# fukangl/SMG-multimodal-grasping

Hardware: AMD Instinct MI355X
Metric: affordance fwd+bwd passes/sec (16-rot 224^2 RGB-D) (higher is better)
Workload: dtype f32; 1 GPU; 16 rot x 224^2 (S=640): fwd + Huber + bwd + Adam per GPU per step; reinforcement_net style 0; 17 trunk passes; fp32; leg=headline, rotations=16, input_size=640, parallelism=dp1

## Files before the change

### smg-multimodal-grasping_amd/csrc/backward.hip

```cpp
#include "engine.h"

int do_backward(smg_engine* e, const smg_net* net, const float* dq, hipStream_t st, int phases, bool elem_head) {
    if (!e->have_fwd) return fail(-22, "smg_backward without a preceding smg_forward");
    if (!net->grads) return fail(-22, "net.grads is NULL");
    if (phases == 2 && !e->bw_phase0_done)
        return fail(-22, "smg_backward_phase(1) must follow smg_backward_phase(0) of the same forward");
    if ((phases & 1) && e->bw_phase0_done)
        return fail(-22, "smg_backward / smg_backward_phase(0) while the second half of a two-phase backward is still due (run phase 1 or a new forward)");
    const Layout& L = *e->L;
    const TrunkRef& T = L.trunk[e->f_trunk];
    const HeadRef& Hd = L.head[e->f_head];
    const int NS = e->f_streams, NP = e->f_pairs;
    const float* P = net->params;
    float* Gr = net->grads;
    const Plane p4 = e->p_blk[3];
    const bool ph_a = phases & 1, ph_b = phases & 2;
    if (ph_a) {
        for (int r = 0; r < kStatRep; ++r) HIP_OK(hipMemsetAsync(e->bstat + (size_t)r * kStatRepStride, 0, 2 * e->bstat_span * sizeof(double), st));
    }
    const bool split16 = e->prec == 0 && kSplitOp == 3;
    if (ph_a && split16) HIP_OK(hipMemsetAsync(e->gamax, 0, (size_t)e->gamax_words * sizeof(unsigned), st));
    const hipStream_t s2 = (e->prof || e->serialize) ? st : e->side;
    auto fork = [&](hipEvent_t ev) -> int {
        HIP_OK(hipEventRecord(ev, st));
        HIP_OK(hipStreamWaitEvent(s2, ev, 0));
        return 0;
    };
    const bool gs_materialised = split16 || NS > 4;
    auto gs_on_side = [&](const Plane& pl) { return split16 && !e->generic3x3 && pl.HW <= 1600 && NS <= 4; };
    auto fused_gsrc = [&](int b, const DenseLayerRef& d) {
        return grad_src(e, e->G[b], kBlockCtot[b], e->X[b], kBlockCtot[b], e->st_X[b], d.cin, nullptr);
    };
    auto launch_gs_apply = [&](int b, int i, hipStream_t cs, float* GSb, const GradSrc& fused) {
        const Plane pl = e->p_blk[b];
        BnBwdApplyArgs a{};
        a.src = fused; a.src.xtab = stat_table(e, e->sx_tab[b], e->max_streams, kBlockCtot[b], T.layers[b][i].cin);
        a.pl = pl; a.C = kGrowth;
        a.out = GSb; a.ldo = kGrowth; a.amax = split16 ? gamax_of(e, b, i, 0) : nullptr;
        PREC_DISPATCH(e, launch_kernel(e, bn_bwd_apply_kernel<PREC>, dim3((pl.HWp + bn_apply_rows(PREC) - 1) / bn_apply_rows(PREC), NS), dim3(256), 0, cs,
                                       K_OTHER, 0, ESZ(e) * NS * pl.HW * 3 * kGrowth, false, a));
    };

    auto norm1_src = [&](int b, int i, int c0) {
        const DenseLayerRef& d = T.layers[b][i];
        return act_src(e, e->X[b], kBlockCtot[b], e->st_X[b], c0, P + d.n1.w, P + d.n1.b, stat_table(e, e->sx_tab[b], e->max_streams, kBlockCtot[b]), asc_n1(e, b, i));
    };
    auto norm2_src = [&](int b, int i) {
        const DenseLayerRef& d = T.layers[b][i];
        return act_src(e, el(e, e->Bt, e->bt_off[b][i]), kBottleneck, e->st_Bt[b][i], 0, P + d.n2.w, P + d.n2.b,
                       !e->generic3x3 ? stat_table(e, e->sb_tab[b][i], e->max_streams, kBottleneck) : StatTab{}, asc_n2(e, b, i));
    };

    PartialTiles tiles(e->part_floats, NS, e->deterministic);

    if (ph_a) {
    {
        ValueBwdArgs a;
        a.h1 = head_norm1_src(e, Hd, P); a.p4 = p4; a.w2p = e->packed_f + e->pk_head1;
        a.dq = dq; a.out_ch = e->head_out; a.OH = e->OH; a.OW = e->OW; a.dh1 = e->DH1;
        a.st = stat_sink_bwd(e, e->st_H1, 0); a.aff = affine_sink(Gr, Hd.n1); a.dw2 = Gr + Hd.c1.w;
        const bool dense = !elem_head && (e->head_bwd == 2 || (e->head_bwd == 0 && e->f_dense_dq));
        if (!dense) {
// ... 149 lines not shown
        }
        HIP_OK(hipMemcpyAsync(buf, src, (size_t)elems * (e->prec ? 2 : 4), hipMemcpyDeviceToDevice, st));
        e->dbg_snap_prec = e->prec; n = elems;
        return 0;
    };
    const bool pooled_tail = e->prec == 0 && e->f_stem1 && !e->stem_plane_tail && (NS > 4 || e->deterministic);
    for (int b = ph_a ? 3 : 0; b >= (ph_b ? 0 : 1); --b) {
        e->prof_stage = b;
        const Plane pl = e->p_blk[b];
        const int Ct = kBlockCtot[b];
        if (e->dbg_stop == b * 100 + 50) return debug_stop();
        if (b == 0 && pooled_tail) {
            StemMomArgs a;
            a.img = e->img4; a.pi = e->p_img; a.ps = e->p_stem; a.part = e->mom_part;
            a.tiles_x = stem_mom_tiles_x(e->p_stem); a.n_tiles = stem_mom_tiles(e->p_stem); a.tiles_per_wg = kMomTilesPerWg;
            if (fork(e->ev_misc)) return -5;
            e->prof_stage = -1;
            launch_kernel(e, stem_moments_kernel, dim3(e->mom_groups, NS), dim3(256), 0, s2, K_OTHER, 0, 0, false, a);
            launch_kernel(e, stem_moments_sum_kernel, dim3((kMomOut + 255) / 256, NS), dim3(256), 0, s2, K_OTHER, 0, 0, false,
                          (const float*)e->mom_part, e->mom_groups, e->mom);
            e->prof_stage = b;
        }
        for (int i = (int)T.layers[b].size() - 1; i >= 0; --i) {
            const DenseLayerRef& d = T.layers[b][i];
            float* bt = el(e, e->Bt, e->bt_off[b][i]);
            const ActSrc n2 = norm2_src(b, i);
            const StatSink n2st = stat_sink_bwd(e, e->st_Bt[b][i], 0);
            const LayerBuf lb = buf_of(b, i);
            float* GSb = lb.GS;
            float* D2b = lb.D2;
            static_assert(kRing % 3 == 0 && kRing > 3, "the sparse ring wait covers three slots at a time");
            if (lb.ring >= kRing && lb.ring % 3 == 0) HIP_OK(hipStreamWaitEvent(st, e->ev_side[(lb.ring + 2) % kRing], 0));
            GradSrc gsrc = fused_gsrc(b, d);
            if (e->generic3x3 || (gs_materialised && !gs_on_side(pl))) {
                launch_gs_apply(b, i, st, GSb, gsrc);
                if (gs_materialised) gsrc = grad_done(GSb, kGrowth, gamax_of(e, b, i, 0));
            }
            if (!e->generic3x3) {
                Halo3x3DgradArgs a;
                a.g = gsrc; a.pl = pl; a.C = kBottleneck; a.m = n2;
                a.dst = split16 ? e->DY2 : D2b; a.st = n2st;
                a.wu = e->packed_u + e->pk_hd[b][i];
                const double flops = 2.0 * NS * pl.HW * 9 * kBottleneck * kGrowth;
                const double bytes = ESZ(e) * NS * pl.HW * (kGrowth + 2 * kBottleneck);
                if (halo_tile(pl, NS) == 16) {
                    a.tiles_x = (pl.W + 15) / 16; a.cg_per_wg = kBottleneck / 32;
                    if (pl.H % 16 || pl.W % 16) {
                        PREC_DISPATCH(e, launch_kernel(e, conv3x3_halo_dgrad_kernel<16, PREC, true>, dim3(((pl.H + 15) / 16) * a.tiles_x, NS), dim3(256),
                                                       HaloDgradSGeo<16, PREC>::smem_bytes(kBottleneck), st, K_D3, flops, bytes, true, a));
                    } else {
                        PREC_DISPATCH(e, launch_kernel(e, conv3x3_halo_dgrad_kernel<16, PREC>, dim3((pl.H / 16) * a.tiles_x, NS), dim3(256),
                                                       HaloDgradSGeo<16, PREC>::smem_bytes(kBottleneck), st, K_D3, flops, bytes, true, a));
                    }
                } else {
                    a.tiles_x = (pl.W + 7) / 8; a.cg_per_wg = 1;
                    PREC_DISPATCH(e, launch_kernel(e, conv3x3_halo_dgrad_kernel<8, PREC>, dim3(((pl.H + 7) / 8) * a.tiles_x, NS, kBottleneck / 64), dim3(256),
                                                   HaloDgradSGeo<8, PREC>::smem_bytes(kBottleneck), st, K_D3, flops, bytes, true, a));
                }
            } else {
                auto run = [&](auto tag) {
                    using Cfg = decltype(tag);
                    BwdDataP<Cfg, true, E_STORE, false> p{};
                    p.gs = grad_done(GSb, kGrowth); p.pa = pl; p.KA = kGrowth;
                    p.wp = e->packed_u + e->pk_g3d[b][i]; p.K8tot = 9 * kGrowth / 8; p.ldn = kBottleneck; p.wcol0 = 0; p.N = kBottleneck;
                    p.m = n2; p.pm = pl;
                    p.dst = split16 ? e->DY2 : D2b; p.ldd = kBottleneck; p.dcoff = 0;
                    p.st = n2st; p.aff = affine_sink(Gr, d.n2);
                    launch_gemm(e, st, p, dim3(NS * pl.HWp / Cfg::BM, kBottleneck / Cfg::BN), K_D3, 2.0 * NS * pl.HW * 9 * kBottleneck * kGrowth,
                                ESZ(e) * NS * pl.HW * (kGrowth + 2 * kBottleneck));
                };
                if (pl.HWp % 128 == 0) run(CfgP128x128{}); else run(CfgP64x128{});
            }
            const GradSrc dy2 = grad_src(e, split16 ? e->DY2 : D2b, kBottleneck, bt, kBottleneck, e->st_Bt[b][i], 0, P + d.n2.w,
                                         !e->generic3x3 ? stat_table(e, e->sb_tab[b][i], e->max_streams, kBottleneck) : StatTab{});
            if (split16) {
// ... 182 lines not shown
```

### smg-multimodal-grasping_amd/csrc/engine.h

```cpp
#pragma once
#include <hip/hip_runtime.h>

#include <algorithm>
#include <cmath>
#include <cstdio>
#include <cstdlib>
#include <cstring>
#include <string>
#include <type_traits>
#include <vector>

#include "../../include/smg_hip.h"
#include "elem.cuh"
#include "scene.cuh"
#include "gemm.cuh"
#include "halo.cuh"
#include "ws.cuh"
#include "wsw.cuh"
#include "plan.h"

using namespace smg;

int smg_fail(int code, const std::string& msg);
static inline int fail(int code, const std::string& msg) { return smg_fail(code, msg); }
// ... 45 lines not shown
struct smg_engine {
    int device = 0, S = 0, max_streams = 0, max_pairs = 0, head_out = 1;
    Plane p_img, p_stem, p_blk[4];
    int OH = 1, OW = 1;
    const Layout* L = nullptr;

    float* img4 = nullptr; float* stem = nullptr; float* X[4] = {}; float* Bt = nullptr; int64_t bt_floats = 0;
    std::vector<int64_t> bt_off[4];
    unsigned char* argmax = nullptr;
    float* F = nullptr; float* H1 = nullptr;
    float* G[4] = {}; float* GS[kRing] = {}; float* D2[kRing] = {}; float* part = nullptr; int64_t part_floats = 0;
    float* DY2 = nullptr; float* D2S[kRing] = {};
    hipStream_t side = nullptr; hipEvent_t ev_gs[kRing] = {}, ev_d2[kRing] = {}, ev_side[kRing] = {}, ev_misc = nullptr, ev_end = nullptr; float* DY0 = nullptr; float* DH1 = nullptr; float* DF = nullptr;
    double* fstat = nullptr; int64_t fstat_span = 0;
    double* bstat = nullptr; int64_t bstat_span = 0;
    float* dbscr = nullptr; int db_total = 0; int db_off[4][24] = {}; int db_toff[3] = {}; struct DbSeg* d_dbseg = nullptr; int n_dbseg = 0;
    StatArr st_stem, st_X[4], st_F, st_H1; std::vector<StatArr> st_Bt[4];
    u32x4* packed_u = nullptr; int64_t packed_units = 0;
    float* packed_f = nullptr; int64_t packed_floats = 0;
    PackDesc* d_pack = nullptr; std::vector<PackDesc> h_pack[3]; std::vector<PackDesc> h_pack_head[3];
    int pack_stride = 0, bnupd_stride = 0, n_bnupd = 0;
    int64_t pk_conv0 = 0, pk_conv0_1 = 0, pk_head0 = 0, pk_hd0 = 0, pk_head1 = 0;
    std::vector<int64_t> pk_c1[4], pk_d1[4], pk_g3f[4], pk_g3d[4], pk_hf[4], pk_hd[4]; int64_t pk_t[3] = {}, pk_td[3] = {};
    int max_pack = 0;
    float* asc = nullptr; ActScaleDesc* d_asc = nullptr; int n_asc = 0;
    unsigned* gamax = nullptr; int64_t gamax_words = 0;
    float* stab = nullptr; int64_t stab_floats = 0;
    int64_t sx_tab[4] = {}, sb_tab[4][24] = {}, sf_tab = 0;
    BnUpdDesc* d_bnupd = nullptr;
    bool have_fwd = false; int f_trunk = 0, f_head = 0, f_streams = 0, f_pairs = 0;
    bool bw_phase0_done = false;
    bool f_dense_dq = false;
    int head_bwd = 0;
    bool f_stem1 = false;
    int* d_stream_image = nullptr; int* d_stream_rot = nullptr; int* d_pair_a = nullptr; int* d_pair_b = nullptr;
    int* d_seq_t = nullptr; int* d_seq_h = nullptr; int* d_user_ptr = nullptr; int* d_user_pair = nullptr; int* d_user_slot = nullptr;
    float* d_affine = nullptr;
    float* scene_val = nullptr; int* scene_idx = nullptr; int scene_tiles = 0;
    double* scene_lpart = nullptr;
    double* scene_gpart = nullptr; int* scene_cnt = nullptr;
    int* d_stage = nullptr; int* h_stage[2] = {}; hipEvent_t ev_stage[2] = {}; int stage_ints = 0, stage_turn = 0;
    int so_image = 0, so_rot = 0, so_pa = 0, so_pb = 0, so_seq_t = 0, so_seq_h = 0, so_uptr = 0, so_upair = 0, so_uslot = 0, so_aff = 0, so_ma = 0, so_mb = 0, so_adam = 0;
    bool capturing = false; int* h_stage_g = nullptr; hipEvent_t ev_graph = nullptr, ev_gin = nullptr; hipStream_t gstream = nullptr; struct StepGraph* step_graph = nullptr;
    int64_t workspace_bytes = 0;
    int n_cu = 256;
    int prec = 0;
    bool serialize = false;
    bool deterministic = false;
    bool generic3x3 = false, generic_c1 = false, generic_w1 = false, stem_plane_tail = false;
    float* stemv = nullptr; float* mom_part = nullptr; double* mom = nullptr; int mom_groups = 0;
    int dbg_stop = -1;
    float* dbg_gsnap = nullptr; int64_t dbg_gsnap_floats = 0; int64_t dbg_gsnap_n = 0;
    float* dbg_dy2 = nullptr; int64_t dbg_dy2_floats = 0; int64_t dbg_dy2_n = 0;
    int dbg_snap_prec = -1;
    bool prof = false; std::vector<ProfRec> recs; std::vector<hipEvent_t> ev_pool;
    double prof_ms[5][K_COUNT] = {}; int64_t prof_n[5][K_COUNT] = {}; double prof_flops[5][K_COUNT] = {}; double prof_bytes[5][K_COUNT] = {}; int prof_stage = -1;
    int launch_rc = 0;
};

constexpr int kMomTilesPerWg = 8;
static inline int stem_mom_tiles_x(const Plane& ps) { return (ps.W + kMomT - 1) / kMomT; }
static inline int stem_mom_tiles(const Plane& ps) { return stem_mom_tiles_x(ps) * ((ps.H + kMomT - 1) / kMomT); }
static inline int stem_mom_groups(const Plane& ps) { return (stem_mom_tiles(ps) + kMomTilesPerWg - 1) / kMomTilesPerWg; }

static Plane make_plane(int H, int W) {
    Plane p; p.H = H; p.W = W; p.HW = H * W;
// ... 243 lines not shown
```

### smg-multimodal-grasping_amd/csrc/engine.hip

```cpp
#include "engine.h"

static thread_local std::string g_err;
int smg_fail(int code, const std::string& msg) { g_err = msg; return code; }

static int zero_typed_buffers(smg_engine* e) {
    const int NS = e->max_streams;
    for (int b = 0; b < 4; ++b) {
        const size_t n = (size_t)NS * e->p_blk[b].HWp * kBlockCtot[b] * sizeof(float);
        HIP_OK(hipMemset(e->X[b], 0, n));
        HIP_OK(hipMemset(e->G[b], 0, n));
    }
    HIP_OK(hipMemset(e->Bt, 0, (size_t)e->bt_floats * sizeof(float)));
    for (int k = 0; k < kRing; ++k) {
        HIP_OK(hipMemset(e->D2[k], 0, (size_t)NS * e->p_blk[0].HWp * kBottleneck * sizeof(float)));
        HIP_OK(hipMemset(e->GS[k], 0, (size_t)NS * e->p_blk[0].HWp * kGrowth * sizeof(float)));
    }
    HIP_OK(hipMemset(e->DY2, 0, (size_t)NS * e->p_blk[0].HWp * kBottleneck * sizeof(float)));
    HIP_OK(hipDeviceSynchronize());
    return 0;
}

static int engine_build(smg_engine* e) {
    const Layout& L = *e->L;
    const int NS = e->max_streams, NP = e->max_pairs;
    const int S = e->S;
    const int H1 = (S - 1) / 2 + 1, H2 = (H1 - 1) / 2 + 1;
    e->p_img = make_plane(S, S);
    e->p_stem = make_plane(H1, H1);
    int h = H2;
    for (int b = 0; b < 4; ++b) { e->p_blk[b] = make_plane(h, h); h /= 2; }
    e->OH = e->OW = e->p_blk[3].H - kHeadKernel + 1;
    if (e->OH < 1) return fail(-22, "input_size too small for the 20x20 value head");

    if (getenv("SMG_SERIALIZE")) e->serialize = true;
    const int cross = getenv("SMG_CROSSCHECK") ? atoi(getenv("SMG_CROSSCHECK")) : 0;
    e->generic3x3 = cross & 1; e->generic_c1 = cross & 2; e->generic_w1 = cross & 4; e->stem_plane_tail = cross & 8;

    ALLOC(e->img4, (int64_t)NS * e->p_img.HWp * 4);
    ALLOC(e->stem, (int64_t)NS * e->p_stem.HWp * 64);
    ALLOC(e->DY0, (int64_t)NS * e->p_stem.HWp * 64);
    ALLOC(e->argmax, (int64_t)NS * e->p_blk[0].HWp * 64);
    e->stemv = e->DY0;
    e->mom_groups = stem_mom_groups(e->p_stem);
    ALLOC(e->mom_part, (int64_t)NS * e->mom_groups * kMomVals);
    ALLOC(e->mom, (int64_t)NS * kMomOut);
    int64_t bt_total = 0;
    for (int b = 0; b < 4; ++b) {
        ALLOC(e->X[b], (int64_t)NS * e->p_blk[b].HWp * kBlockCtot[b]);
        ALLOC(e->G[b], (int64_t)NS * e->p_blk[b].HWp * kBlockCtot[b]);
        for (int i = 0; i < kBlockLayers[b]; ++i) {
            e->bt_off[b].push_back(bt_total);
            bt_total += (int64_t)NS * e->p_blk[b].HWp * kBottleneck;
        }
    }
    ALLOC(e->Bt, bt_total);
    for (int k = 0; k < kRing; ++k) {
        ALLOC(e->D2[k], (int64_t)NS * e->p_blk[0].HWp * kBottleneck);
        ALLOC(e->GS[k], (int64_t)NS * e->p_blk[0].HWp * kGrowth);
        ALLOC(e->D2S[k], (int64_t)NS * (e->p_blk[0].HWp / kScaleBlock));
        HIP_OK(hipEventCreateWithFlags(&e->ev_gs[k], hipEventDisableTiming));
        HIP_OK(hipEventCreateWithFlags(&e->ev_d2[k], hipEventDisableTiming));
        HIP_OK(hipEventCreateWithFlags(&e->ev_side[k], hipEventDisableTiming));
    }
    ALLOC(e->DY2, (int64_t)NS * e->p_blk[0].HWp * kBottleneck);
    e->bt_floats = bt_total;
    if (int rc = zero_typed_buffers(e)) return rc;
    e->scene_tiles = (int)(((int64_t)(S / 2) * (S / 2) + kSceneTile - 1) / kSceneTile);
    ALLOC(e->scene_val, (int64_t)kSceneMaps * e->scene_tiles);
    ALLOC(e->scene_idx, (int64_t)kSceneMaps * e->scene_tiles);
// ... 181 lines not shown
            e->n_bnupd = (int)v.size();
            HIP_OK(hipMemcpy(e->d_bnupd + (t * 3 + hd) * e->bnupd_stride, v.data(), v.size() * sizeof(BnUpdDesc), hipMemcpyHostToDevice));
        }

    const int R = NS > NP ? NS : NP;
    int so = 0;
    auto carve_i = [&](int n) { int at = so; so += (n + 3) / 4 * 4; return at; };
    e->so_image = carve_i(NS); e->so_rot = carve_i(NS); e->so_pa = carve_i(NP); e->so_pb = carve_i(NP);
    e->so_seq_t = carve_i(4 * R + 16); e->so_seq_h = carve_i(4 * R + 16);
    e->so_uptr = carve_i(NS + 1); e->so_upair = carve_i(2 * NP); e->so_uslot = carve_i(2 * NP);
    e->so_aff = carve_i(6 * NS); e->so_ma = carve_i(NS); e->so_mb = carve_i(NS);
    e->so_adam = carve_i(4);
    e->stage_ints = so;
    ALLOC(e->d_stage, so);
    e->d_stream_image = e->d_stage + e->so_image; e->d_stream_rot = e->d_stage + e->so_rot;
    e->d_pair_a = e->d_stage + e->so_pa; e->d_pair_b = e->d_stage + e->so_pb;
    e->d_seq_t = e->d_stage + e->so_seq_t; e->d_seq_h = e->d_stage + e->so_seq_h;
    e->d_user_ptr = e->d_stage + e->so_uptr; e->d_user_pair = e->d_stage + e->so_upair; e->d_user_slot = e->d_stage + e->so_uslot;
    e->d_affine = (float*)(e->d_stage + e->so_aff);
    for (int k = 0; k < 2; ++k) {
        HIP_OK(hipHostMalloc((void**)&e->h_stage[k], (size_t)so * sizeof(int), hipHostMallocDefault));
        HIP_OK(hipEventCreateWithFlags(&e->ev_stage[k], hipEventDisableTiming));
    }
    HIP_OK(hipHostMalloc((void**)&e->h_stage_g, (size_t)so * sizeof(int), hipHostMallocDefault));
    memset(e->h_stage_g, 0, (size_t)so * sizeof(int));
    HIP_OK(hipEventCreateWithFlags(&e->ev_graph, hipEventDisableTiming));
    HIP_OK(hipEventCreateWithFlags(&e->ev_gin, hipEventDisableTiming));
    HIP_OK(hipStreamCreateWithFlags(&e->gstream, hipStreamNonBlocking));
    return 0;
}

struct StepKey {
    const void* params; const void* grads; const void* bufs; const void* nbt;
    int trunk_id, head_id, n_streams, n_pairs, n_images, hm_size, n_seq_t, n_seq_h, n_masks, loss_mode, prec, deterministic, head_bwd;
    const void* images; const void* heightmaps; const void* masks; double mean, stdv;
    const void* labels; const void* q; const void* loss; const void* dq; const void* m; const void* v; float lr, b1, b2, eps;
    hipStream_t stream;
    bool operator==(const StepKey& o) const { return memcmp(this, &o, sizeof(StepKey)) == 0; }
};
struct StepGraph {
    StepKey key; bool warm = false;
    hipGraph_t graph = nullptr; hipGraphExec_t exec = nullptr;
};
static void step_graph_drop(smg_engine* e) {
    if (!e->step_graph) return;
    if (e->step_graph->exec) (void)hipGraphExecDestroy(e->step_graph->exec);
    if (e->step_graph->graph) (void)hipGraphDestroy(e->step_graph->graph);
    delete e->step_graph;
    e->step_graph = nullptr;
}
static void adam_scalars(const smg_adam* a, int step, float* sc) {
    const double bc1 = 1.0 - std::pow((double)a->beta1, step), bc2 = 1.0 - std::pow((double)a->beta2, step);
    sc[0] = (float)((double)a->lr / bc1);
    sc[1] = (float)std::sqrt(bc2);
}
static int step_body(smg_engine* e, const smg_net* net, int trunk_id, int head_id, const smg_batch* B, int loss_mode, const float* labels,
                     float* q, float* loss, float* dq, const smg_adam* adam, hipStream_t st) {
    const Layout& L = *e->L;
    const int64_t t0 = L.trunk[trunk_id].p_begin, tn = L.trunk[trunk_id].p_feat_end - t0, h0 = L.head[head_id].p_begin, hn = L.head[head_id].p_end - h0;
    HIP_OK(hipMemsetAsync(net->grads + t0, 0, (size_t)tn * sizeof(float), st));
    HIP_OK(hipMemsetAsync(net->grads + h0, 0, (size_t)hn * sizeof(float), st));
    if (int rc = do_forward(e, net, trunk_id, head_id, B, q, st)) return rc;
    const int per_pair = e->head_out * e->OH * e->OW;
    hipLaunchKernelGGL(loss_kernel, dim3((B->n_pairs + 63) / 64), dim3(64), 0, st, loss_mode, (const float*)q, labels, B->n_pairs, per_pair, loss, dq);
    e->f_dense_dq = false;
    if (int rc = do_backward(e, net, dq, st, 3, true)) return rc;
    const float* sc = reinterpret_cast<const float*>(e->d_stage + e->so_adam);
// ... 472 lines not shown
    return do_backward(e, net, dq_dev, (hipStream_t)stream);
}

int smg_backward_phase(smg_engine* e, const smg_net* net, const float* dq_dev, void* stream, int phase) {
    if (!e || !net || !dq_dev) return fail(-22, "NULL argument");
    if (phase != 0 && phase != 1) return fail(-22, "phase must be 0 or 1");
    HIP_OK(hipSetDevice(e->device));
    return do_backward(e, net, dq_dev, (hipStream_t)stream, phase == 0 ? 1 : 2);
}

int smg_layout_trunk_split(int head_out, int trunk_id, int64_t* offset) {
    if (trunk_id < 0 || trunk_id > 2 || !offset) return fail(-22, "trunk_id");
    *offset = layout_for(head_out).trunk[trunk_id].tnorm[0].w;
    return 0;
}

int smg_train_step_graph(smg_engine* e, const smg_net* net, int trunk_id, int head_id, const smg_batch* B, int loss_mode,
                         const float* labels_dev, float* q_out_dev, float* loss_out_dev, float* dq_dev, const smg_adam* adam, void* stream) {
    if (!e || !net || !B || !labels_dev || !q_out_dev || !loss_out_dev || !dq_dev || !adam) return fail(-22, "NULL argument");
    if (!net->params || !net->grads || !net->bufs || !net->nbt || !adam->m || !adam->v) return fail(-22, "net / optimizer arrays are NULL");
    if (trunk_id < 0 || trunk_id > 2 || head_id < 0 || head_id > 2) return fail(-22, "trunk_id / head_id out of range");
    if (loss_mode != 0 && loss_mode != 1) return fail(-22, "loss mode must be 0 (Huber) or 1 (cross entropy)");
    if (loss_mode == 1 && e->head_out != 3) return fail(-22, "cross-entropy loss needs a 3-class head");
    if (adam->step_trunk < 1 || adam->step_head < 1) return fail(-22, "Adam step counts are 1-based");
    if (e->prof || e->serialize) return fail(-22, "smg_train_step_graph: not while profiling / serialised (the graph spans two streams)");
    HIP_OK(hipSetDevice(e->device));
    if (int rc = validate_batch(e, B)) return rc;
    hipStream_t caller = (hipStream_t)stream, st = e->gstream;
    StepKey key;
    memset(&key, 0, sizeof(key));
    key.params = net->params; key.grads = net->grads; key.bufs = net->bufs; key.nbt = net->nbt;
    key.trunk_id = trunk_id; key.head_id = head_id; key.n_streams = B->n_streams; key.n_pairs = B->n_pairs; key.n_images = B->n_images;
    key.hm_size = B->hm_size; key.n_seq_t = B->bn_seq_trunk ? B->n_bn_seq_trunk : 0; key.n_seq_h = B->bn_seq_head ? B->n_bn_seq_head : 0;
    key.n_masks = B->masks_dev ? B->n_masks : 0; key.loss_mode = loss_mode; key.prec = e->prec; key.deterministic = e->deterministic; key.head_bwd = e->head_bwd;
    key.images = B->images_nchw_dev; key.heightmaps = B->heightmaps_dev; key.masks = B->masks_dev; key.mean = B->image_mean; key.stdv = B->image_std;
    key.labels = labels_dev; key.q = q_out_dev; key.loss = loss_out_dev; key.dq = dq_dev; key.m = adam->m; key.v = adam->v;
    key.lr = adam->lr; key.b1 = adam->beta1; key.b2 = adam->beta2; key.eps = adam->eps; key.stream = caller;
    HIP_OK(hipEventSynchronize(e->ev_graph));
    if (e->step_graph && !(e->step_graph->key == key)) step_graph_drop(e);
    if (!e->step_graph) { e->step_graph = new StepGraph(); e->step_graph->key = key; }
    StepGraph* g = e->step_graph;
    fill_stage(e, B, e->h_stage_g);
    float* sc = reinterpret_cast<float*>(e->h_stage_g + e->so_adam);
    adam_scalars(adam, adam->step_trunk, sc);
    adam_scalars(adam, adam->step_head, sc + 2);
    HIP_OK(hipEventRecord(e->ev_gin, caller));
    HIP_OK(hipStreamWaitEvent(st, e->ev_gin, 0));
    e->capturing = true;
    int rc = 0;
    if (!g->warm) {
        rc = step_body(e, net, trunk_id, head_id, B, loss_mode, labels_dev, q_out_dev, loss_out_dev, dq_dev, adam, st);
        g->warm = rc == 0;
    } else {
        if (!g->exec) {
            hipError_t err = hipStreamBeginCapture(st, hipStreamCaptureModeRelaxed);
            if (err != hipSuccess) { e->capturing = false; return fail(-5, std::string("hipStreamBeginCapture: ") + hipGetErrorString(err)); }
            rc = step_body(e, net, trunk_id, head_id, B, loss_mode, labels_dev, q_out_dev, loss_out_dev, dq_dev, adam, st);
            err = hipStreamEndCapture(st, &g->graph);
            if (rc == 0 && err != hipSuccess) rc = fail(-5, std::string("hipStreamEndCapture: ") + hipGetErrorString(err));
            if (rc == 0) {
                err = hipGraphInstantiate(&g->exec, g->graph, nullptr, nullptr, 0);
                if (err != hipSuccess) rc = fail(-5, std::string("hipGraphInstantiate: ") + hipGetErrorString(err));
            }
            if (rc) { e->capturing = false; step_graph_drop(e); return rc; }
        }
        hipError_t err = hipGraphLaunch(g->exec, st);
        if (err != hipSuccess) rc = fail(-5, std::string("hipGraphLaunch: ") + hipGetErrorString(err));
// ... 1 lines not shown
        e->f_stem1 = B->heightmaps_dev != nullptr; e->f_dense_dq = false;
    }
    e->capturing = false;
    if (rc == 0) {
        HIP_OK(hipEventRecord(e->ev_graph, st));
        HIP_OK(hipStreamWaitEvent(caller, e->ev_graph, 0));
    }
    return rc;
}

int smg_engine_set_precision(smg_engine* e, int precision) {
    if (!e) return fail(-22, "engine is NULL");
    if (precision < 0 || precision > 2) return fail(-22, "precision must be 0 (fp32 storage, fp32-class split products), 1 (bf16 storage) or 2 (fp16 activations, bf16 gradients)");
    if (precision && e->generic3x3) return fail(-22, "SMG_CROSSCHECK=1 (the generic implicit-GEMM 3x3 path) exists in the fp32-class mode only");
    if (precision != e->prec) {
        HIP_OK(hipSetDevice(e->device));
        HIP_OK(hipDeviceSynchronize());
        if (int rc = zero_typed_buffers(e)) return rc;
    }
    e->prec = precision;
    step_graph_drop(e);
    e->have_fwd = false;
    e->bw_phase0_done = false;
    return 0;
}

int smg_engine_set_option(smg_engine* e, const char* name, int value) {
    if (!e || !name) return fail(-22, "NULL argument");
    const std::string s(name);
    if (s == "deterministic") { e->deterministic = value != 0; return 0; }
    if (s == "head_bwd") {
        if (value < 0 || value > 2) return fail(-22, "head_bwd must be 0 (follow the mark of smg_loss_map / smg_loss_map_ce), 1 (per-element form) or 2 (dense form)");
        e->head_bwd = value; return 0;
    }
    if (s == "serialize") { e->serialize = value != 0; return 0; }
    if (s == "debug_stop") { e->dbg_stop = value; return 0; }
    return fail(-22, "unknown engine option '" + s + "'");
}

int smg_heightmap(const double* depth_img_dev, int h, int w, const double* intrinsics3x3, const double* cam_pose4x4,
                  const double* inv_homography3x3, int out_w, int out_h, double* out_dev, void* stream) {
    if (!depth_img_dev || !intrinsics3x3 || !cam_pose4x4 || !inv_homography3x3 || !out_dev || h < 1 || w < 1 || out_w < 1 || out_h < 1)
        return fail(-22, "bad heightmap arguments");
    hipPointerAttribute_t attr;
    HIP_OK(hipPointerGetAttributes(&attr, depth_img_dev));
    HIP_OK(hipSetDevice(attr.device));
    HeightmapArgs a;
    a.depth = depth_img_dev; a.h = h; a.w = w;
    a.fx = intrinsics3x3[0]; a.fy = intrinsics3x3[4]; a.cx = intrinsics3x3[2]; a.cy = intrinsics3x3[5];
    a.r20 = cam_pose4x4[8]; a.r21 = cam_pose4x4[9]; a.r22 = cam_pose4x4[10]; a.t2 = cam_pose4x4[11];
    for (int i = 0; i < 9; ++i) a.mi[i] = inv_homography3x3[i];
    a.out = out_dev; a.ow = out_w; a.oh = out_h;
    hipLaunchKernelGGL(heightmap_warp_kernel, dim3((out_w + 255) / 256, out_h), dim3(256), 0, (hipStream_t)stream, a);
    HIP_OK(hipGetLastError());
    return 0;
}

int smg_argmax(const float* values_dev, int n, int* idx_out_dev, float* val_out_dev, void* stream) {
    if (!values_dev || !idx_out_dev || !val_out_dev || n < 1) return fail(-22, "bad argmax arguments");
    hipPointerAttribute_t attr;
    HIP_OK(hipPointerGetAttributes(&attr, values_dev));
    HIP_OK(hipSetDevice(attr.device));
    hipLaunchKernelGGL(argmax_kernel, dim3(1), dim3(256), 0, (hipStream_t)stream, values_dev, n, idx_out_dev, val_out_dev);
    HIP_OK(hipGetLastError());
    return 0;
}
// ... 115 lines not shown
        if (!host_out) return n;
        const int ns_out = (int)std::min<int64_t>(NS, cap / per_stream);
        n = ns_out * per_stream;
        HIP_OK(hipSetDevice(e->device));
        HIP_OK(hipStreamSynchronize((hipStream_t)stream));
        if (e->prec != 0) {
            std::vector<unsigned short> raw((size_t)n);
            HIP_OK(hipMemcpy(raw.data(), gs ? e->GS[slot] : e->D2[slot], raw.size() * sizeof(unsigned short), hipMemcpyDeviceToHost));
            widen16(raw.data(), n, false, host_out);
            return n;
        }
        if (gs || kSplitOp != 3) {
            HIP_OK(hipMemcpy(host_out, gs ? e->GS[slot] : e->D2[slot], n * sizeof(float), hipMemcpyDeviceToHost));
            return n;
        }
        std::vector<unsigned short> u((size_t)ns_out * per_stream * 2);
        std::vector<float> inv((size_t)NS * (pl.HWp / kScaleBlock));
        HIP_OK(hipMemcpy(u.data(), e->D2[slot], u.size() * sizeof(unsigned short), hipMemcpyDeviceToHost));
        HIP_OK(hipMemcpy(inv.data(), e->D2S[slot], inv.size() * sizeof(float), hipMemcpyDeviceToHost));
        auto h2f = [](unsigned h) -> double {
            const int ex = (h >> 10) & 31, man = h & 1023;
            const double v = ex == 0 ? std::ldexp((double)man, -24) : (ex == 31 ? (man ? NAN : INFINITY) : std::ldexp((double)(man | 1024), ex - 25));
            return (h & 0x8000u) ? -v : v;
        };
        for (int sn = 0; sn < ns_out; ++sn)
            for (int k8 = 0; k8 < kD2K8; ++k8)
                for (int p = 0; p < pl.HWp; ++p) {
                    const size_t uh = ((((size_t)sn * 2 + 0) * kD2K8 + k8) * pl.HWp + p) * 8, ul = ((((size_t)sn * 2 + 1) * kD2K8 + k8) * pl.HWp + p) * 8;
                    const double iv = inv[(size_t)sn * (pl.HWp / kScaleBlock) + p / kScaleBlock];
                    for (int j = 0; j < 8; ++j)
                        host_out[((size_t)sn * pl.HWp + p) * kBottleneck + 8 * k8 + j] = (float)((h2f(u[uh + j]) + h2f(u[ul + j])) * iv);
                }
        return n;
    } else if (s == "asc") {
        src = e->asc; n = 2 * e->n_asc;
    } else if (s.size() >= 6 && s.substr(0, 5) == "fs_bt") {
        int b = 0, i = 0;
        if (std::sscanf(name, "fs_bt%d_%d", &b, &i) != 2 || b < 1 || b > 4 || i < 1 || i > kBlockLayers[b - 1]) return fail(-22, "bad fs_bt name");
        n = (int64_t)4 * NS * kBottleneck;
        if (!host_out) return n;
        if (cap < n) return fail(-22, "fs_bt: buffer too small");
        HIP_OK(hipSetDevice(e->device));
        HIP_OK(hipStreamSynchronize((hipStream_t)stream));
        HIP_OK(hipMemcpy(host_out, fsum(e, e->st_Bt[b - 1][i - 1]), (size_t)NS * kBottleneck * sizeof(double), hipMemcpyDeviceToHost));
        HIP_OK(hipMemcpy(host_out + 2 * NS * kBottleneck, fsq(e, e->st_Bt[b - 1][i - 1]), (size_t)NS * kBottleneck * sizeof(double), hipMemcpyDeviceToHost));
        return n;
    } else return fail(-22, "unknown debug buffer");
    if (!host_out) return n;
    if (cap < n) n = cap;
    HIP_OK(hipSetDevice(e->device));
    HIP_OK(hipStreamSynchronize((hipStream_t)stream));
    const bool typed = e->prec != 0 && (s[0] == 'x' || s[0] == 'g' || s.substr(0, 2) == "bt" || s == "dy2");
    if (!typed) {
        HIP_OK(hipMemcpy(host_out, src, n * sizeof(float), hipMemcpyDeviceToHost));
        return n;
    }
    std::vector<unsigned short> raw((size_t)n);
    HIP_OK(hipMemcpy(raw.data(), src, n * sizeof(unsigned short), hipMemcpyDeviceToHost));
    const bool f16 = e->prec == 2 && s[0] != 'g' && s != "dy2";
    widen16(raw.data(), n, f16, host_out);
    return n;
}

int smg_profile_enable(smg_engine* e, int on) {
    if (!e) return fail(-22, "engine is NULL");
    e->prof = on != 0;
// ... 40 lines not shown
```

### smg-multimodal-grasping_amd/csrc/halo.cuh

```cuda
#pragma once
#include "gemm.cuh"

namespace smg {

constexpr int kHaloFwdWaves = 2, kHaloWgradWaves = 2;

template <int TS>
struct HaloGeo {
    static_assert(TS == 16 || TS == 8, "tile side");
    static constexpr int T = TS, W = TS + 2, PX = W * W, NPIX = TS * TS;
    static constexpr int MT = NPIX == 256 ? 2 : 1;
    static constexpr int WQ = NPIX / (32 * MT);
    static constexpr int WX = 4 / WQ;
    static constexpr int ROWS = 32 / TS;
    static constexpr int RP = MT + 2;
    static constexpr int RSTEP = TS == 16 ? 2 : 0;
    __device__ static __forceinline__ int row(int wq, int m, int i) { return (wq * MT + m) * ROWS + i / TS; }
    __device__ static __forceinline__ int col(int i) { return i % TS; }
    __device__ static __forceinline__ int rowi(int wq, int m, int i) { return TS == 16 ? 4 * wq + m + 2 * (i / TS) : row(wq, m, i); }
    __device__ static __forceinline__ int pair0(int wq) { return 4 * wq; }
};

template <int B, int N, class F>
__device__ __forceinline__ void sfor(F&& f) {
// ... 351 lines not shown
    double* red = reinterpret_cast<double*>(smem);
    __syncthreads();
    if (half == 0) { red[wave * 32 + l31] = s; red[128 + wave * 32 + l31] = ss; }
    __syncthreads();
    if (t < 64) {
        const int q = t >> 5, c = t & 31;
        const double tot = red[q * 128 + c] + red[q * 128 + 32 + c] + red[q * 128 + 64 + c] + red[q * 128 + 96 + c];
        stat_sink_add<S_FWD>(a.st, n, c, q, tot);
    }
    if (trace) { trace[4] = smg_stamp(); trace[6] = __builtin_amdgcn_s_memrealtime(); }
}


__device__ __forceinline__ void grad_src_params(const GradSrc& s, int n, int hw, float* gp) {
    const int t = threadIdx.x;
    if (s.x && t < 32) {
        const GradCoef f = grad_src_coef(s, n, t, 1.0 / (double)hw);
        gp[t] = f.a;
        gp[32 + t] = f.q1;
        gp[64 + t] = f.mean;
        gp[96 + t] = f.k;
    }
}

struct Halo3x3DgradArgs {
    GradSrc g; Plane pl;
    const u32x4* wu;
    ActSrc m;
    int C;
    void* dst;
    StatSink st;
    int tiles_x;
    int cg_per_wg;
};

template <int TS, int PREC> struct HaloDgradSGeo : HaloGeo<TS> {
    using G = HaloGeo<TS>;
    static constexpr int NP = np_of(bwd_op(PREC));
    static constexpr int BU = NP * 4 * 32;
    static constexpr int LDH = G::PX;
    static constexpr int A_UNITS = NP * 4 * LDH;
    static constexpr int A_N = (G::PX * (PREC ? 4 : 8) + 255) / 256;
    static constexpr int NCW = G::WX;
    static constexpr int ST = TS == 8 ? 1 : 3;
    static constexpr int B_UNITS = NCW * ST * BU;
    static constexpr int B_N = (B_UNITS + 255) / 256;
    static constexpr int B_PAD = B_N * 256;
    __host__ __device__ static constexpr int smem_bytes(int C) { return (A_UNITS + 2 * B_PAD) * 16 + (4 * C + 256 + 128) * 4; }
};

template <int TS, int PREC = 0, bool RAG = false>
static __global__ __launch_bounds__(256, TS == 8 ? 4 : 2) void conv3x3_halo_dgrad_kernel(const Halo3x3DgradArgs a) {
    constexpr bool kEdge = TS == 8 || RAG;
    using G = HaloDgradSGeo<TS, PREC>;
    using GT = grd_t<PREC>;
    using XT = act_t<PREC>;
    constexpr int OP = bwd_op(PREC), NP = G::NP, HDS_BU = G::BU, GSZ = GT::size, XSZ = XT::size, E = 16 / GSZ, SPP = 32 / E;
    constexpr int MT = G::MT, NCW = G::NCW, A_N = G::A_N, B_N = G::B_N, LDH = G::LDH;
    constexpr bool kRegFrag = TS == 16 && OP == 3;
    constexpr bool kDma = kRegFrag && G::NCW == 1 && G::B_UNITS % 256 == 0 && 2 * G::B_PAD <= G::A_UNITS;
    extern __shared__ __attribute__((aligned(16))) float smem[];
    char* As = reinterpret_cast<char*>(smem);
    char* Bs = As + G::A_UNITS * 16;
    float* prm = reinterpret_cast<float*>(Bs + 2 * G::B_PAD * 16);
    const int t = threadIdx.x, lane = t & 63, wave = t >> 6, l31 = lane & 31, half = lane >> 5;
    const int wq = wave % G::WQ, wc = wave / G::WQ;
// ... 49 lines not shown
        if (!a.g.x) {
            unsigned m = 0;
#pragma unroll
            for (int r = 0; r < kAmaxRep / 4; ++r) m = max(max(m, max(am4[r].x, am4[r].y)), max(am4[r].z, am4[r].w));
            gsc = scale_of_max(m);
            gsc.inv *= pack_inv_scale(a.wu);
        }
    }
    constexpr int ST = G::ST;
    u32x4 rb[B_N];
    unsigned b_voff[B_N];
#pragma unroll
    for (int i = 0; i < B_N; ++i) {
        const int idx = t + 256 * i;
        const int j = min(idx / (ST * HDS_BU), NCW - 1), rem = idx - j * ST * HDS_BU;
        b_voff[i] = 16u * (unsigned)(j * 9 * HDS_BU + rem);
    }
    auto g_load = [&](int stage) {
        const int cg = cg0 + stage / (3 * SPR), tap0 = (stage % (3 * SPR)) * ST;
#pragma unroll
        for (int i = 0; i < B_N; ++i) rb[i] = bload_u4(a.wu, kWholeBuf, b_voff[i], 16u * (unsigned)((cg * NCW * 9 + tap0) * HDS_BU));
    };
    {
#ifdef SMG_TRACE_INIT
        if (trace) trace[1] = smg_stamp();
#endif
        __syncthreads();
#ifdef SMG_TRACE_INIT
        asm volatile("s_waitcnt vmcnt(0)" ::: "memory");
        if (trace) trace[2] = smg_stamp();
#endif
        if constexpr (OP == 3) {
            if (x_n) {
                float vmax = 0.f;
#pragma unroll
                for (int i = 0; i < A_N; ++i) {
                    const int idx = t + 256 * i;
                    const int hp = idx / SPP, q = idx % SPP;
                    const int hy = hp / G::W, hx = hp - hy * G::W;
                    const int iy = y0 - 1 + hy, ix = x0 - 1 + hx;
                    const bool ok = idx < G::PX * SPP && (unsigned)iy < (unsigned)a.pl.H && (unsigned)ix < (unsigned)a.pl.W;
                    const float4 v = ok ? affine2(rv[i], rx[i], gp + 4 * (q % 8), 32) : zero4();
                    rv[i] = v;
                    vmax = fmaxf(fmaxf(vmax, fmaxf(fabsf(v.x), fabsf(v.y))), fmaxf(fabsf(v.z), fabsf(v.w)));
                }
#pragma unroll
                for (int o = 32; o > 0; o >>= 1) vmax = fmaxf(vmax, __shfl_xor(vmax, o));
                float* red = prm + 4 * C;
                if (lane == 0) red[wave] = vmax;
                __syncthreads();
                vmax = fmaxf(fmaxf(red[0], red[1]), fmaxf(red[2], red[3]));
                if (vmax > 0.f) gsc = scale_of_max(__float_as_uint(vmax));
                gsc.inv *= pack_inv_scale(a.wu);
            }
        }
#pragma unroll
        for (int i = 0; i < A_N; ++i) {
            const int idx = t + 256 * i;
            if (idx < G::PX * SPP) {
                const int hp = idx / SPP, q = idx % SPP;
                const int hy = hp / G::W, hx = hp - hy * G::W;
                const int iy = y0 - 1 + hy, ix = x0 - 1 + hx;
                const bool ok = (unsigned)iy < (unsigned)a.pl.H && (unsigned)ix < (unsigned)a.pl.W;
                if constexpr (E == 4) {
                    float4 v = rv[i];
                    if (OP != 3 && x_n) v = affine2(rv[i], rx[i], gp + 4 * q, 32);
                    if constexpr (OP == 3) v = mul4(v, gsc.s);
                    if (!ok) v = zero4();
                    const Split4 sp = split4<OP>(v);
#pragma unroll
                    for (int pc = 0; pc < NP; ++pc)
                        *reinterpret_cast<uint2*>(As + ((pc * 4 + (q >> 1)) * LDH + hp) * 16 + (q & 1) * 8) = sp.p[pc];
                } else {
                    u32x4 u = as_u4(rv[i]);
                    if (x_n) u = pack_unit<OP>(affine2(slot_quad<GT>(rv[i], 0), slot_quad<XT>(rx[i], 0), gp + 8 * q, 32),
                                               affine2(slot_quad<GT>(rv[i], 1), slot_quad<XT>(rx[i], 1), gp + 8 * q + 4, 32));
                    if (!ok) u = u32x4{0u, 0u, 0u, 0u};
                    *reinterpret_cast<u32x4*>(As + (q * LDH + hp) * 16) = u;
                }
            }
        }
    }
    auto s_store = [&](int buf) {
// ... 427 lines not shown
```

Before: 62.24 passes/s.

## Fuse grad-source materialisation into 3x3 halo dgrad for large-tile planes

Adds an option for the 3x3 halo data-gradient kernel to write the BN-backward gradient source (GS) tile interior and its abs-max while it stages its input, in place of a separate bn_bwd_apply launch. This is on by default for 16x16-tile planes when the split16 path is used with more than four streams. It removes one kernel launch and one full read-and-write pass of the gradient per layer. In exchange the dgrad kernel does extra stores and an atomicMax. The change also adds env and setter knobs and a gamax debug readout.

```diff
diff --git a/smg-multimodal-grasping_amd/csrc/backward.hip b/smg-multimodal-grasping_amd/csrc/backward.hip
--- a/smg-multimodal-grasping_amd/csrc/backward.hip
+++ b/smg-multimodal-grasping_amd/csrc/backward.hip
@@ -1,4 +1,7 @@
 #include "engine.h"
+
+constexpr bool kGsFromDgradSmall = false;
+constexpr bool kGsFromDgradBig = true;
 
 int do_backward(smg_engine* e, const smg_net* net, const float* dq, hipStream_t st, int phases, bool elem_head) {
     if (!e->have_fwd) return fail(-22, "smg_backward without a preceding smg_forward");
@@ -28,6 +31,13 @@
     };
     const bool gs_materialised = split16 || NS > 4;
     auto gs_on_side = [&](const Plane& pl) { return split16 && !e->generic3x3 && pl.HW <= 1600 && NS <= 4; };
+    auto gs_from_dgrad = [&](const Plane& pl, int b, int i) {
+        if (!split16 || e->generic3x3 || NS <= 4 || e->gs_form == 1) return false;
+        if (e->gs_form == 5) return e->dbg_stop == b * 100 + i;
+        const bool small = halo_tile(pl, NS) == 8;
+        return e->gs_form == 2 || (e->gs_form == 3 && small) || (e->gs_form == 4 && !small) || (e->gs_form == 0 && kGsFromDgradSmall && small)
+               || (e->gs_form == 0 && kGsFromDgradBig && !small);
+    };
     auto fused_gsrc = [&](int b, const DenseLayerRef& d) {
         return grad_src(e, e->G[b], kBlockCtot[b], e->X[b], kBlockCtot[b], e->st_X[b], d.cin, nullptr);
     };
@@ -243,7 +253,10 @@
             static_assert(kRing % 3 == 0 && kRing > 3, "the sparse ring wait covers three slots at a time");
             if (lb.ring >= kRing && lb.ring % 3 == 0) HIP_OK(hipStreamWaitEvent(st, e->ev_side[(lb.ring + 2) % kRing], 0));
             GradSrc gsrc = fused_gsrc(b, d);
-            if (e->generic3x3 || (gs_materialised && !gs_on_side(pl))) {
+            const bool from_dgrad = gs_from_dgrad(pl, b, i);
+            if (from_dgrad) {
+                gsrc.xtab = stat_table(e, e->sx_tab[b], e->max_streams, kBlockCtot[b], d.cin);
+            } else if (e->generic3x3 || (gs_materialised && !gs_on_side(pl))) {
                 launch_gs_apply(b, i, st, GSb, gsrc);
                 if (gs_materialised) gsrc = grad_done(GSb, kGrowth, gamax_of(e, b, i, 0));
             }
@@ -252,6 +265,7 @@
                 a.g = gsrc; a.pl = pl; a.C = kBottleneck; a.m = n2;
                 a.dst = split16 ? e->DY2 : D2b; a.st = n2st;
                 a.wu = e->packed_u + e->pk_hd[b][i];
+                if (from_dgrad) { a.gs_out = GSb; a.gs_amax = gamax_of(e, b, i, 0); }
                 const double flops = 2.0 * NS * pl.HW * 9 * kBottleneck * kGrowth;
                 const double bytes = ESZ(e) * NS * pl.HW * (kGrowth + 2 * kBottleneck);
                 if (halo_tile(pl, NS) == 16) {
diff --git a/smg-multimodal-grasping_amd/csrc/engine.h b/smg-multimodal-grasping_amd/csrc/engine.h
--- a/smg-multimodal-grasping_amd/csrc/engine.h
+++ b/smg-multimodal-grasping_amd/csrc/engine.h
@@ -101,6 +101,7 @@
     bool bw_phase0_done = false;
     bool f_dense_dq = false;
     int head_bwd = 0;
+    int gs_form = 0;
     bool f_stem1 = false;
     int* d_stream_image = nullptr; int* d_stream_rot = nullptr; int* d_pair_a = nullptr; int* d_pair_b = nullptr;
     int* d_seq_t = nullptr; int* d_seq_h = nullptr; int* d_user_ptr = nullptr; int* d_user_pair = nullptr; int* d_user_slot = nullptr;
diff --git a/smg-multimodal-grasping_amd/csrc/engine.hip b/smg-multimodal-grasping_amd/csrc/engine.hip
--- a/smg-multimodal-grasping_amd/csrc/engine.hip
+++ b/smg-multimodal-grasping_amd/csrc/engine.hip
@@ -35,6 +35,10 @@
     if (getenv("SMG_SERIALIZE")) e->serialize = true;
     const int cross = getenv("SMG_CROSSCHECK") ? atoi(getenv("SMG_CROSSCHECK")) : 0;
     e->generic3x3 = cross & 1; e->generic_c1 = cross & 2; e->generic_w1 = cross & 4; e->stem_plane_tail = cross & 8;
+    if (const char* gf = getenv("SMG_GS_FORM")) {
+        e->gs_form = atoi(gf);
+        if (e->gs_form < 0 || e->gs_form > 5) return fail(-22, "SMG_GS_FORM must be 0..5 (engine.h: gs_form)");
+    }
 
     ALLOC(e->img4, (int64_t)NS * e->p_img.HWp * 4);
     ALLOC(e->stem, (int64_t)NS * e->p_stem.HWp * 64);
@@ -282,7 +286,7 @@
 
 struct StepKey {
     const void* params; const void* grads; const void* bufs; const void* nbt;
-    int trunk_id, head_id, n_streams, n_pairs, n_images, hm_size, n_seq_t, n_seq_h, n_masks, loss_mode, prec, deterministic, head_bwd;
+    int trunk_id, head_id, n_streams, n_pairs, n_images, hm_size, n_seq_t, n_seq_h, n_masks, loss_mode, prec, deterministic, head_bwd, gs_form;
     const void* images; const void* heightmaps; const void* masks; double mean, stdv;
     const void* labels; const void* q; const void* loss; const void* dq; const void* m; const void* v; float lr, b1, b2, eps;
     hipStream_t stream;
@@ -821,7 +825,7 @@
     key.params = net->params; key.grads = net->grads; key.bufs = net->bufs; key.nbt = net->nbt;
     key.trunk_id = trunk_id; key.head_id = head_id; key.n_streams = B->n_streams; key.n_pairs = B->n_pairs; key.n_images = B->n_images;
     key.hm_size = B->hm_size; key.n_seq_t = B->bn_seq_trunk ? B->n_bn_seq_trunk : 0; key.n_seq_h = B->bn_seq_head ? B->n_bn_seq_head : 0;
-    key.n_masks = B->masks_dev ? B->n_masks : 0; key.loss_mode = loss_mode; key.prec = e->prec; key.deterministic = e->deterministic; key.head_bwd = e->head_bwd;
+    key.n_masks = B->masks_dev ? B->n_masks : 0; key.loss_mode = loss_mode; key.prec = e->prec; key.deterministic = e->deterministic; key.head_bwd = e->head_bwd; key.gs_form = e->gs_form;
     key.images = B->images_nchw_dev; key.heightmaps = B->heightmaps_dev; key.masks = B->masks_dev; key.mean = B->image_mean; key.stdv = B->image_std;
     key.labels = labels_dev; key.q = q_out_dev; key.loss = loss_out_dev; key.dq = dq_dev; key.m = adam->m; key.v = adam->v;
     key.lr = adam->lr; key.b1 = adam->beta1; key.b2 = adam->beta2; key.eps = adam->eps; key.stream = caller;
@@ -889,6 +893,11 @@
     if (s == "head_bwd") {
         if (value < 0 || value > 2) return fail(-22, "head_bwd must be 0 (follow the mark of smg_loss_map / smg_loss_map_ce), 1 (per-element form) or 2 (dense form)");
         e->head_bwd = value; return 0;
+    }
+    if (s == "gs_form") {
+        if (value < 0 || value > 5)
+            return fail(-22, "gs_form must be 0 (the policy), 1 (an apply launch on the chain), 2 (the 3x3 data gradient writes GS) or, for A/B runs and tests, 3 / 4 (8 x 8- / 16 x 16-tile planes only) / 5 (the debug_stop layer only)");
+        e->gs_form = value; return 0;
     }
     if (s == "serialize") { e->serialize = value != 0; return 0; }
     if (s == "debug_stop") { e->dbg_stop = value; return 0; }
@@ -1070,6 +1079,11 @@
                         host_out[((size_t)sn * pl.HWp + p) * kBottleneck + 8 * k8 + j] = (float)((h2f(u[uh + j]) + h2f(u[ul + j])) * iv);
                 }
         return n;
+    } else if (s.size() >= 8 && s.substr(0, 6) == "gamax_") {
+        int b = 0, i = 0;
+        if (std::sscanf(name + 6, "%d_%d", &b, &i) != 2 || b < 1 || b > 4 || i < 1 || i > kBlockLayers[b - 1]) return fail(-22, "bad gamax name");
+        if (!e->gamax || e->prec != 0) return fail(-22, "gamax: gradient maxima are recorded in precision mode 0 only");
+        src = reinterpret_cast<const float*>(gamax_of(e, b - 1, i - 1, 0)); n = (int64_t)NS * kAmaxRep;
     } else if (s == "asc") {
         src = e->asc; n = 2 * e->n_asc;
     } else if (s.size() >= 6 && s.substr(0, 5) == "fs_bt") {
diff --git a/smg-multimodal-grasping_amd/csrc/halo.cuh b/smg-multimodal-grasping_amd/csrc/halo.cuh
--- a/smg-multimodal-grasping_amd/csrc/halo.cuh
+++ b/smg-multimodal-grasping_amd/csrc/halo.cuh
@@ -407,6 +407,8 @@
     StatSink st;
     int tiles_x;
     int cg_per_wg;
+    float* gs_out = nullptr;
+    unsigned* gs_amax = nullptr;
 };
 
 template <int TS, int PREC> struct HaloDgradSGeo : HaloGeo<TS> {
@@ -522,7 +524,8 @@
 #endif
         if constexpr (OP == 3) {
             if (x_n) {
-                float vmax = 0.f;
+                const bool gs_store = a.gs_out && blockIdx.z == 0;
+                float vmax = 0.f, cmax = 0.f;
 #pragma unroll
                 for (int i = 0; i < A_N; ++i) {
                     const int idx = t + 256 * i;
@@ -532,13 +535,27 @@
                     const bool ok = idx < G::PX * SPP && (unsigned)iy < (unsigned)a.pl.H && (unsigned)ix < (unsigned)a.pl.W;
                     const float4 v = ok ? affine2(rv[i], rx[i], gp + 4 * (q % 8), 32) : zero4();
                     rv[i] = v;
-                    vmax = fmaxf(fmaxf(vmax, fmaxf(fabsf(v.x), fabsf(v.y))), fmaxf(fabsf(v.z), fabsf(v.w)));
+                    const float m4 = fmaxf(fmaxf(fabsf(v.x), fabsf(v.y)), fmaxf(fabsf(v.z), fabsf(v.w)));
+                    vmax = fmaxf(vmax, m4);
+                    if (gs_store && ok && (unsigned)(hy - 1) < (unsigned)TS && (unsigned)(hx - 1) < (unsigned)TS) {
+                        *reinterpret_cast<float4*>(a.gs_out + ((int64_t)n * a.pl.HWp + iy * a.pl.W + ix) * 32 + 4 * q) = v;
+                        cmax = fmaxf(cmax, m4);
+                    }
                 }
 #pragma unroll
                 for (int o = 32; o > 0; o >>= 1) vmax = fmaxf(vmax, __shfl_xor(vmax, o));
                 float* red = prm + 4 * C;
                 if (lane == 0) red[wave] = vmax;
+                if (gs_store) {
+#pragma unroll
+                    for (int o = 32; o > 0; o >>= 1) cmax = fmaxf(cmax, __shfl_xor(cmax, o));
+                    if (lane == 0) red[4 + wave] = cmax;
+                }
                 __syncthreads();
+                if (gs_store && t == 0) {
+                    cmax = fmaxf(fmaxf(red[4], red[5]), fmaxf(red[6], red[7]));
+                    if (cmax > 0.f) atomicMax(a.gs_amax + (int64_t)n * kAmaxRep + (blockIdx.x % kAmaxRep), __float_as_uint(cmax));
+                }
                 vmax = fmaxf(fmaxf(red[0], red[1]), fmaxf(red[2], red[3]));
                 if (vmax > 0.f) gsc = scale_of_max(__float_as_uint(vmax));
                 gsc.inv *= pack_inv_scale(a.wu);
```

Result: no change. 62.72 passes/s, median of 6 (+0.8%).
